# AI4Science-WestlakeU/safediffcon

Hardware: AMD Instinct MI355X
Metric: sampled control trajectories/sec (1000-step DDPM) (higher is better)
Workload: dtype f32; 1 GPU; C4: 2D smoke Unet3D_with_Conv3D dim=64 (1,2,4) state (B,32,7,64,64), B=64 per GPU, guided 1000-step DDPM, conformal quantile on; batch_per_gpu=64, global_batch=64, step=U-Net + guidance + posterior update of the whole batch, one hipGraph replay, parallelism=batch-sharded x1, no data-path collective, conv_precision=fp32

## Files before the change

### safediffcon_amd/csrc/sdc_conv.h

```cpp
#pragma once
#include "sdc_common.h"
#include <cstdlib>
#include <type_traits>

namespace sdcconv {


#ifdef SDC_KERNEL_EXPERIMENTS
inline int exp_env(const char* name) { const char* v = getenv(name); return v ? atoi(v) : 0; }
#else
constexpr int exp_env(const char*) { return 0; }
#endif


constexpr int BK = 16;
constexpr int NT = 256;

typedef float f32x16 __attribute__((ext_vector_type(16)));

typedef const __attribute__((address_space(1))) float* gfloat_p;
__device__ __forceinline__ gfloat_p uniform_ptr(const float* p) {
    const uint64_t u = reinterpret_cast<uint64_t>(p);
    const uint32_t lo = __builtin_amdgcn_readfirstlane((uint32_t)u);
    const uint32_t hi = __builtin_amdgcn_readfirstlane((uint32_t)(u >> 32));
    return (gfloat_p)(((uint64_t)hi << 32) | lo);
}
#define SDC_UNIFORM(v) __builtin_amdgcn_readfirstlane(v)
__device__ __forceinline__ float ld_sv(gfloat_p base, uint32_t byte_off) {
    typedef const __attribute__((address_space(1))) char* gchar_p;
    return *(gfloat_p)((gchar_p)base + byte_off);
}

struct ConvArgs {
    SdcConvDesc d;
    const float* x0;
    const float* x1;
    const float* wp;
    const float* bias;
    const float* res;
    float* y;
    int Ntot;
    int Ktot;
    int Cin;
    int lgD, lgH, lgW;
    int vec2;
    int ydense;
    const float* wg2;
    double* gn_part;
    int gn_G, gn_cpg, gn_nparts, gn_S;
    int ksplit;
    int64_t ypart_elems;
};

__device__ __forceinline__ int xcd_tile(int bid, int ntiles) {
    return (ntiles & 7) == 0 ? (bid & 7) * (ntiles >> 3) + (bid >> 3) : bid;
}

constexpr int W2_SK = 8;
constexpr int W2_BM = 64;
constexpr int W2_TILES = 64;
constexpr int W2_NBUF = 2;
constexpr int W2_ASZ = 16 * W2_SK * W2_BM, W2_BSZ = 16 * W2_SK * W2_TILES;
constexpr int W3S_TILES = 32;

inline int64_t span5(const int64_t* st, int b, int c, int dd, int h, int w) {
    return (int64_t)(b - 1) * st[0] + (int64_t)(c - 1) * st[1] + (int64_t)(dd - 1) * st[2] + (int64_t)(h - 1) * st[3] + (int64_t)(w - 1) * st[4];
}

bool wg2_ok(const SdcConvDesc& d, bool small);
bool wg3_ok(const SdcConvDesc& d, bool small);
int launch_wg2(const ConvArgs& a, hipStream_t s);
int wg2_ksplit(const SdcConvDesc& d);
int launch_wg3(const ConvArgs& a, hipStream_t s);
bool wg3s_ok(const SdcConvDesc& d, bool small);
bool wg2s_ok(const SdcConvDesc& d, bool small);
int launch_wg2s(const ConvArgs& a, hipStream_t s);
int launch_wg3s(const ConvArgs& a, hipStream_t s);

int f16_kc(int kD, int kH, int kW);
bool f16_faster(const SdcConvDesc& d);
bool f16_ok(const SdcConvDesc& d);
int f16_gnparts(const SdcConvDesc& d, int G);
const char* f16_name(const SdcConvDesc& d);
int launch_f16(const ConvArgs& a, const _Float16* wh, hipStream_t s, const int32_t* gexp = nullptr);
int pack_f16_tail(const float* w, float* tail, int64_t gap, int Cout, int Cin, int kD, int kH, int kW, hipStream_t s);

struct StemShape { int Hs, NG, NR, itemsB; size_t lds; };
StemShape stem_shape(const SdcConvDesc& d);
int launch_stem_f16(const SdcConvDesc& d, const float* x, const _Float16* wh, const float* bias, float* y, hipStream_t s);

int launch_stem_x3(const SdcConvDesc& d, const float* x, const __bf16* wb, const float* bias, float* y, hipStream_t s);

bool gemm_x3_covers(const SdcConvDesc& d);
int launch_gemm_x3(const SdcConvDesc& d, const float* x, const __bf16* wb, const float* bias, float* y, hipStream_t s);

int pw_x3_block(int K, int Cout);
int launch_pw_x3(const ConvArgs& a, hipStream_t s);

}
```

### safediffcon_amd/csrc/sdc_conv_gemm_x3.hip

```cpp
#include "sdc_conv.h"
#include "sdc_split3.h"

using namespace sdcconv;

namespace {

constexpr int GX_BM = 64, GX_BN = 256, GX_NT = 256;

struct GemmX3Args {
    const float* x;
    const __bf16* wb;
    const float* bias;
    float* y;
    int64_t xs[5], ys[5];
    int NP, oD, Cout, oH, W, lgW, iH, iW, lgIW;
    int pH, pW;
    int Hs, GR, NR, RP;
    int IMG;
    int RT, nrows, ntiles, mtiles, itemsB, nst;
    int plane;
};

template <int FORM> struct GxForm;
template <> struct GxForm<0> { static constexpr int TAPS = 16, NCB = 1, SS = 4, SH = 2, NPAR = 2; };
template <> struct GxForm<1> { static constexpr int TAPS = 4, NCB = 2, SS = 8, SH = 1, NPAR = 1; };
template <> struct GxForm<2> { static constexpr int TAPS = 1, NCB = 4, SS = 4, SH = 1, NPAR = 1; };

template <int FORM, int ITB>
__global__ __launch_bounds__(GX_NT) __attribute__((amdgpu_waves_per_eu(1))) SDC_NO_DS_MERGE void conv_gemm_x3_kernel(const GemmX3Args a) {
    using F = GxForm<FORM>;
    constexpr int TAPS = F::TAPS, NCB = F::NCB, SS = F::SS, SH = F::SH;
    constexpr int KS = NCB * TAPS;
    constexpr int NSUB = KS / SS;
    constexpr bool PREF = ITB <= 9;
    static_assert(NSUB * SS == KS, "whole sub-stages");
    constexpr int APC = SS * GX_BM * 32;
    constexpr int ASZ = 3 * APC;
    constexpr int NIA = 3 * SS * GX_BM * 2;
    constexpr int ITA = (NIA + GX_NT - 1) / GX_NT;
    extern __shared__ __attribute__((aligned(16))) char lds[];

    const int tid = threadIdx.x, lane = tid & 63, wave = tid >> 6;
    const int l31 = lane & 31, lh = lane >> 5;
    const int W = a.W, RP = a.RP;
    const int IMG = a.IMG, BIMG = 2 * NCB * IMG;
    const int PIMG = a.NR * RP * 16;
    const int logical = xcd_tile(blockIdx.x, a.ntiles * a.mtiles);
    const int mt = logical % a.mtiles, nt = logical / a.mtiles;
    const int m0 = mt * GX_BM;
    const int r0 = nt * a.RT;
    const int plane0 = r0 / a.oH, oh0 = r0 - plane0 * a.oH;

    int64_t bb[ITB];
    int bdst[ITB];
    bool bok[ITB];
#pragma unroll
    for (int k = 0; k < ITB; ++k) {
        const int it = tid + k * GX_NT;
        const int w = it & (a.iW - 1);
        const int rest = it >> a.lgIW;
        const int q = rest / a.NR, sr = rest - q * a.NR;
        const int g = sr / a.GR, sq = sr - g * a.GR;
        const int pl = plane0 + g, ih = SH * (g == 0 ? oh0 : 0) - a.pH + sq;
        const bool ok = it < a.itemsB && pl < a.NP && ih >= 0 && ih < a.iH;
        const int b = ok ? pl / a.oD : 0, od = ok ? pl % a.oD : 0, ihc = ok ? ih : 0;
        bok[k] = ok;
        bb[k] = (int64_t)b * a.xs[0] + (int64_t)od * a.xs[2] + (int64_t)ihc * a.xs[3] + (int64_t)w * a.xs[4]
                + (int64_t)((q >> 1) * 16 + (q & 1) * 8) * a.xs[1];
        int col;
        if (FORM == 0) col = (w & 1) * (PIMG / 16) + sr * RP + (w >> 1) + 1;
        else if (FORM == 1) col = sr * RP + w + 1;
        else col = sr * RP + w;
        bdst[k] = ASZ + q * IMG + col * 16;
    }
    int aoff[ITA];
#pragma unroll
    for (int k = 0; k < ITA; ++k) {
        const int it = tid + k * GX_NT;
        const int p = it / (SS * 2 * GX_BM), q = it - p * (SS * 2 * GX_BM);
        aoff[k] = it < NIA ? p * a.plane + mt * (a.nst * KS * GX_BM * 16) + q * 8 : 0;
    }

    float bv[ITB][8];
    uint4 av[ITA];
    auto load_a = [&](int st, int sub) {
        const int wst = (st * KS + sub * SS) * (GX_BM * 16);
#pragma unroll
        for (int k = 0; k < ITA; ++k) {
            uint4 v = make_uint4(0u, 0u, 0u, 0u);
            if (tid + k * GX_NT < NIA) v = *reinterpret_cast<const uint4*>(a.wb + wst + aoff[k]);
            av[k] = v;
        }
    };
    auto load_b = [&](int st) {
        const int64_t co = (int64_t)st * (NCB * 16) * a.xs[1];
#pragma unroll
        for (int k = 0; k < ITB; ++k) {
            const float* q = a.x + bb[k] + co;
#pragma unroll
            for (int i = 0; i < 8; ++i) { bv[k][i] = bok[k] ? *q : 0.0f; q += a.xs[1]; }
        }
    };
    auto store_a = [&]() {
#pragma unroll
        for (int k = 0; k < ITA; ++k)
            if (tid + k * GX_NT < NIA) *reinterpret_cast<uint4*>(lds + (tid + k * GX_NT) * 16) = av[k];
    };
    auto store_b = [&]() {
#pragma unroll
        for (int k = 0; k < ITB; ++k) {
            if (tid + k * GX_NT < a.itemsB) {
                bf16x8 h, m, l;
                split3x8(bv[k], h, m, l);
                *reinterpret_cast<bf16x8*>(lds + bdst[k]) = h;
                *reinterpret_cast<bf16x8*>(lds + bdst[k] + BIMG) = m;
                *reinterpret_cast<bf16x8*>(lds + bdst[k] + 2 * BIMG) = l;
            }
        }
    };

    if (FORM != 2) {
        const int nrows = 3 * 2 * NCB * F::NPAR * a.NR;
        for (int e = tid; e < 2 * nrows; e += GX_NT) {
            const int row = e >> 1;
            *reinterpret_cast<uint4*>(lds + ASZ + (row * RP + ((e & 1) ? RP - 1 : 0)) * 16) = make_uint4(0u, 0u, 0u, 0u);
        }
    }

    int bB[2];
#pragma unroll
    for (int j = 0; j < 2; ++j) {
        const int p = wave * 64 + 32 * j + l31;
        const bool pok = (p >> a.lgW) < a.RT && r0 + (p >> a.lgW) < a.nrows;
        const int rl = pok ? p >> a.lgW : 0, col = pok ? p & (W - 1) : 0;
        const int row = r0 + rl, pl = row / a.oH, oh = row - pl * a.oH, g = pl - plane0;
        const int slot = g * a.GR + SH * (oh - (g == 0 ? oh0 : 0));
        bB[j] = ASZ + (slot * RP + col + (FORM == 1 ? 1 - a.pW : 0)) * 16 + lh * IMG;
    }
    const int aoffr = l31 * 32 + 16 * lh;
    const int rowb = RP * 16;

    f32x16 acc[2][2], sm[2][2];
#pragma unroll
    for (int i = 0; i < 2; ++i)
#pragma unroll
        for (int j = 0; j < 2; ++j)
#pragma unroll
            for (int r = 0; r < 16; ++r) {
                acc[i][j][r] = 0.0f;
                sm[i][j][r] = 0.0f;
            }

    load_a(0, 0);
    if (PREF) load_b(0);
    for (int st = 0; st < a.nst; ++st) {
#pragma unroll
        for (int sub = 0; sub < NSUB; ++sub) {
            __syncthreads();
            store_a();
            if (sub == 0) {
                if (!PREF) load_b(st);
                store_b();
            }
            __syncthreads();
            if (sub + 1 < NSUB) load_a(st, sub + 1);
            else if (st + 1 < a.nst) {
                load_a(st + 1, 0);
                if (PREF) load_b(st + 1);
            }
#pragma unroll
            for (int sl = 0; sl < SS; ++sl) {
                const int ks = sub * SS + sl;
                const int cbk = ks / TAPS, tap = ks - cbk * TAPS;
                int tb = cbk * 2 * IMG;
                if (FORM == 0) {
                    const int kh = tap >> 2, kw = tap & 3;
                    tb += ((kw + 1) & 1) * PIMG + kh * rowb + ((kw + 1) >> 1) * 16;
                } else if (FORM == 1) {
                    tb += (tap >> 1) * rowb + (tap & 1) * 16;
                }
                bf16x8 af[2][3], bf[2][3];
#pragma unroll
                for (int i = 0; i < 2; ++i)
#pragma unroll
                    for (int p = 0; p < 3; ++p)
                        af[i][p] = *reinterpret_cast<const bf16x8*>(lds + p * APC + (sl * GX_BM + 32 * i) * 32 + aoffr);
#pragma unroll
                for (int j = 0; j < 2; ++j)
#pragma unroll
                    for (int p = 0; p < 3; ++p) bf[j][p] = *reinterpret_cast<const bf16x8*>(lds + bB[j] + tb + p * BIMG);
#pragma unroll
                for (int t = 0; t < 6; ++t)
#pragma unroll
                    for (int i = 0; i < 2; ++i)
#pragma unroll
                        for (int j = 0; j < 2; ++j) {
                            f32x16& c = t < 5 ? sm[i][j] : acc[i][j];
                            c = __builtin_amdgcn_mfma_f32_32x32x16_bf16(af[i][X3_PA[t]], bf[j][X3_PB[t]], c, 0, 0, 0);
                        }
            }
        }
    }

#pragma unroll
    for (int i = 0; i < 2; ++i)
#pragma unroll
        for (int j = 0; j < 2; ++j) acc[i][j] += sm[i][j];
    float bz[2][16];
#pragma unroll
    for (int i = 0; i < 2; ++i)
#pragma unroll
        for (int rr = 0; rr < 16; ++rr) bz[i][rr] = 0.0f;
    if (a.bias) {
#pragma unroll
        for (int i = 0; i < 2; ++i)
#pragma unroll
            for (int rr = 0; rr < 16; ++rr) bz[i][rr] = a.bias[m0 + 32 * i + 4 * lh + (rr & 3) + 8 * (rr >> 2)];
    }
#pragma unroll
    for (int j = 0; j < 2; ++j) {
        const int p = wave * 64 + 32 * j + l31;
        if ((p >> a.lgW) >= a.RT || r0 + (p >> a.lgW) >= a.nrows) continue;
        const int row = r0 + (p >> a.lgW), col = p & (W - 1);
        const int pl = row / a.oH, oh = row - pl * a.oH;
        const int b = pl / a.oD, od = pl - b * a.oD;
        float* yp = a.y + (int64_t)b * a.ys[0] + (int64_t)od * a.ys[2] + (int64_t)oh * a.ys[3] + (int64_t)col * a.ys[4]
                    + (int64_t)(m0 + 4 * lh) * a.ys[1];
#pragma unroll
        for (int i = 0; i < 2; ++i) {
#pragma unroll
            for (int rr = 0; rr < 16; ++rr)
                yp[(int64_t)(32 * i + (rr & 3) + 8 * (rr >> 2)) * a.ys[1]] = acc[i][j][rr] + bz[i][rr];
        }
    }
}

__global__ __launch_bounds__(256) void pack_gemm_x3_kernel(const float* __restrict__ wp, __bf16* __restrict__ out, int Cout, int Cin, int taps,
                                                           int ncb, int64_t n) {
    const int64_t e = (int64_t)blockIdx.x * 256 + threadIdx.x;
    if (e >= n) return;
    const int c16 = (int)(e & 15), col = (int)((e >> 4) & 63);
    int64_t r = e >> 10;
    const int KS = ncb * taps, nst = Cin / (16 * ncb);
    const int ks = (int)(r % KS); r /= KS;
    const int st = (int)(r % nst);
    const int mt = (int)(r / nst);
    const int cbk = ks / taps, tap = ks - cbk * taps;
    const int ci = (st * ncb + cbk) * 16 + c16, co = mt * 64 + col;
    __bf16 ph, pm, pl;
    split3(wp[((int64_t)tap * Cin + ci) * Cout + co], ph, pm, pl);
    out[e] = ph; out[n + e] = pm; out[2 * n + e] = pl;
}

int gx_ncb(int kH, int kW) { return kH == 4 && kW == 4 ? 1 : kH == 2 && kW == 2 ? 2 : kH == 1 && kW == 1 ? 4 : 0; }

struct GxShape { int form, RT, Hs, NG, GR, NR, RP, itemsB, IMG; size_t lds; };

GxShape gx_shape(const SdcConvDesc& d) {
    GxShape s{};
    s.form = d.kH == 4 ? 0 : d.kH == 2 ? 1 : 2;
    const int ncb = gx_ncb(d.kH, d.kW), npar = s.form == 0 ? 2 : 1, sh = s.form == 0 ? 2 : 1;
    const int ss = s.form == 1 ? 8 : 4;
    const int R = GX_BN / d.oW;
    const int maxit = (s.form == 0 ? 12 : 8) * GX_NT;
    auto fill = [&](int ng) {
        s.NG = ng;
        s.GR = sh * (s.Hs - 1) + d.kH;
        s.NR = s.NG * s.GR;
        s.RP = s.form == 0 ? d.iW / 2 + 2 : s.form == 1 ? d.iW + 2 : d.iW;
        s.IMG = npar * s.NR * s.RP * 16;
        s.itemsB = 2 * ncb * s.NR * d.iW;
        s.lds = (size_t)3 * ss * GX_BM * 32 + (size_t)3 * 2 * ncb * s.IMG;
        return s.itemsB <= maxit && s.lds <= 160u * 1024u;
    };
    if (d.oH < R) {
        s.Hs = d.oH;
        int ng = R / d.oH;
        while (!fill(ng) && ng > 1) --ng;
        s.RT = s.NG * d.oH;
    } else {
        s.Hs = R; s.RT = R;
        fill(d.oH % R == 0 ? 1 : 2);
    }
    return s;
}

}

namespace sdcconv {

bool gemm_x3_covers(const SdcConvDesc& d) {
    if (!(d.kD == 1 && d.sD == 1 && d.pD == 0 && d.uD == 1 && d.uH == 1 && d.uW == 1 && d.up_mode == 0 && d.oD == d.iD)) return false;
    if (!(d.B > 0 && d.oD > 0 && d.oH > 0 && d.Cin1 == 0 && d.Cout > 0 && d.Cout % 64 == 0)) return false;
    for (int i = 0; i < 5; ++i)
        if (d.rs[i] != 0 || d.x1s[i] != 0) return false;
    const int ncb = gx_ncb(d.kH, d.kW);
    if (ncb == 0 || d.Cin0 <= 0 || d.Cin0 % (16 * ncb) != 0) return false;
    if (d.kH == 4) {
        if (!(d.sH == 2 && d.sW == 2 && d.pH == 1 && d.pW == 1 && d.iH == 2 * d.oH && d.iW == 2 * d.oW)) return false;
    } else if (d.kH == 2) {
        if (!(d.sH == 1 && d.sW == 1 && (d.pH == 0 || d.pH == 1) && (d.pW == 0 || d.pW == 1) && d.iH == d.oH && d.iW == d.oW)) return false;
    } else {
        if (!(d.sH == 1 && d.sW == 1 && d.pH == 0 && d.pW == 0 && d.iH == d.oH && d.iW == d.oW)) return false;
    }
    if (!(d.oW == 16 || d.oW == 32 || d.oW == 64 || d.oW == 128)) return false;
    const GxShape s = gx_shape(d);
    return s.itemsB <= (s.form == 0 ? 12 : 8) * GX_NT && s.lds <= 160u * 1024u;
}

int launch_gemm_x3(const SdcConvDesc& d, const float* x, const __bf16* wb, const float* bias, float* y, hipStream_t s) {
    SDC_REQUIRE(reinterpret_cast<uintptr_t>(wb) % 16 == 0, SDC_EALIGN, "sdc_conv_gemm_x3: the packed weight buffer must be 16-byte aligned");
    const GxShape sh = gx_shape(d);
    const int ncb = gx_ncb(d.kH, d.kW);
    GemmX3Args a;
    a.x = x; a.wb = wb; a.bias = bias; a.y = y;
    for (int i = 0; i < 5; ++i) { a.xs[i] = d.x0s[i]; a.ys[i] = d.ys[i]; }
    a.NP = d.B * d.oD; a.oD = d.oD; a.Cout = d.Cout; a.oH = d.oH; a.W = d.oW; a.iH = d.iH; a.iW = d.iW;
    a.lgW = d.oW == 16 ? 4 : d.oW == 32 ? 5 : d.oW == 64 ? 6 : 7;
    a.lgIW = d.iW == d.oW ? a.lgW : a.lgW + 1;
    a.pH = d.pH; a.pW = d.pW;
    a.Hs = sh.Hs; a.GR = sh.GR; a.NR = sh.NR; a.RP = sh.RP; a.IMG = sh.IMG;
    const int64_t nrows = (int64_t)d.B * d.oD * d.oH;
    SDC_REQUIRE(nrows * d.oW < (1ll << 31), SDC_EINVAL, "sdc_conv_gemm_x3: too many output positions");
    const int64_t plane = (int64_t)d.kH * d.kW * d.Cin0 * d.Cout;
    SDC_REQUIRE(3 * plane < (1ll << 31), SDC_EINVAL, "sdc_conv_gemm_x3: weight too large");
    a.plane = (int)plane;
    a.nrows = (int)nrows; a.RT = sh.RT;
    a.ntiles = (a.nrows + sh.RT - 1) / sh.RT; a.mtiles = d.Cout / GX_BM;
    a.itemsB = sh.itemsB;
    a.nst = d.Cin0 / (16 * ncb);
    SDC_REQUIRE((int64_t)a.ntiles * a.mtiles < (1ll << 31), SDC_EINVAL, "sdc_conv_gemm_x3: grid too large");
    const dim3 grid((unsigned)(a.ntiles * a.mtiles));
#define GX_LAUNCH(FORM, ITB)                                                                                        \
    do {                                                                                                            \
        static std::atomic<uint64_t> attr{0};                                                                       \
        SDC_LDS_OPTIN(attr, (conv_gemm_x3_kernel<FORM, ITB>), 160 * 1024, "sdc_conv_gemm_x3");                      \
        hipLaunchKernelGGL((conv_gemm_x3_kernel<FORM, ITB>), grid, dim3(GX_NT), sh.lds, s, a);                      \
    } while (0)
    if (sh.form == 0) { if (sh.itemsB <= 9 * GX_NT) GX_LAUNCH(0, 9); else GX_LAUNCH(0, 12); }
    else if (sh.form == 1) { if (sh.itemsB <= 5 * GX_NT) GX_LAUNCH(1, 5); else GX_LAUNCH(1, 8); }
    else GX_LAUNCH(2, 8);
#undef GX_LAUNCH
    return sdc::check_launch("sdc_conv_gemm_x3");
}

}

extern "C" size_t sdc_pack_gemm_x3_bytes(int Cout, int Cin, int kH, int kW) {
    const int ncb = gx_ncb(kH, kW);
    if (ncb == 0 || Cout <= 0 || Cout % 64 != 0 || Cin <= 0 || Cin % (16 * ncb) != 0) return 0;
    return (size_t)3 * kH * kW * Cin * Cout * sizeof(__bf16);
}

extern "C" int sdc_pack_gemm_x3(const float* wp, void* out, int Cout, int Cin, int kH, int kW, void* stream) {
    SDC_REQUIRE(wp && out, SDC_ENULL, "sdc_pack_gemm_x3: null pointer");
    SDC_REQUIRE(sdc_pack_gemm_x3_bytes(Cout, Cin, kH, kW) > 0, SDC_EINVAL,
                "sdc_pack_gemm_x3: taps 4x4, 2x2 or 1x1, Cout a multiple of 64, Cin a multiple of 16 / 32 / 64 (got %dx%d, Cin %d, Cout %d)",
                kH, kW, Cin, Cout);
    const int64_t n = (int64_t)kH * kW * Cin * Cout;
    SDC_REQUIRE(n / 256 + 1 < (1ll << 31), SDC_EINVAL, "sdc_pack_gemm_x3: weight too large");
    hipLaunchKernelGGL(pack_gemm_x3_kernel, dim3((unsigned)((n + 255) / 256)), dim3(256), 0, sdc::as_stream(stream), wp,
                       reinterpret_cast<__bf16*>(out), Cout, Cin, kH * kW, gx_ncb(kH, kW), n);
    return sdc::check_launch("sdc_pack_gemm_x3");
}

static bool gemm_x3_faster(const SdcConvDesc& d) {
    const bool c64 = d.Cin0 == 64 && d.Cout == 64 && d.oH == 32 && d.oW == 32;
    const bool c128 = d.Cin0 == 128 && d.Cout == 128 && d.oH == 16 && d.oW == 16;
    return (d.kH == 4 || d.kH == 2) && (c64 || c128);
}

extern "C" int sdc_conv_gemm_x3_ok(const SdcConvDesc* dp) {
    return dp && gemm_x3_covers(*dp) && gemm_x3_faster(*dp) ? 1 : 0;
}

extern "C" int sdc_conv_gemm_x3(const SdcConvDesc* dp, const float* x, const void* wb, const float* bias, float* y, void* stream) {
    SDC_REQUIRE(dp && x && wb && y, SDC_ENULL, "sdc_conv_gemm_x3: null pointer");
    SDC_REQUIRE(gemm_x3_covers(*dp), SDC_EINVAL, "sdc_conv_gemm_x3: descriptor not covered: %dx%dx%d taps, stride %dx%dx%d, Cin %d+%d, Cout %d, "
                "residual %d, output %dx%dx%d", dp->kD, dp->kH, dp->kW, dp->sD, dp->sH, dp->sW, dp->Cin0, dp->Cin1, dp->Cout, (int)(dp->rs[1] != 0),
                dp->oD, dp->oH, dp->oW);
    return launch_gemm_x3(*dp, x, reinterpret_cast<const __bf16*>(wb), bias, y, sdc::as_stream(stream));
}
```

### safediffcon_amd/csrc/sdc_conv_stem_x3.hip

```cpp
#include "sdc_conv.h"
#include "sdc_conv_stem_tile.h"
#include "sdc_split3.h"

using namespace sdcconv;

namespace {

struct StemX3Args {
    STEM_TILE_ARGS(__bf16, wb)
    int plane;
};

template <int KH, int ITB>
__global__ __launch_bounds__(STEM_NT) __attribute__((amdgpu_waves_per_eu(1))) SDC_NO_DS_MERGE void conv_stem_x3_kernel(const StemX3Args a) {
    constexpr int TAPS = KH * 7;
    constexpr int NS = (TAPS + 1) / 2;
    constexpr int SS = KH == 7 ? 5 : NS;
    constexpr int NSUB = NS / SS;
    static_assert(NSUB * SS == NS, "whole sub-stages");
    constexpr int HH = KH - 1;
    constexpr int APC = SS * STEM_BM * 32;
    constexpr int ASZ = 3 * APC;
    constexpr int NIA = 3 * SS * STEM_BM * 2;
    constexpr int ITA = (NIA + STEM_NT - 1) / STEM_NT;
    extern __shared__ __attribute__((aligned(16))) char lds[];

    const int tid = threadIdx.x, lane = tid & 63, wave = tid >> 6;
    const int l31 = lane & 31, lh = lane >> 5;
    const int W = a.W, RP = W + 6;
    const int BIMG = a.NR * RP * 16;
    const StemTile t = stem_tile(a);
    const int m0 = t.m0, n0 = t.n0, r0 = t.r0, plane0 = t.plane0, oh0 = t.oh0;
    const int GR = a.Hs + HH;

    int64_t bb[ITB];
    int bod[ITB], bdst[ITB];
    bool bok[ITB];
#pragma unroll
    for (int k = 0; k < ITB; ++k) {
        const int it = tid + k * STEM_NT;
        const int w = it & (W - 1);
        const int sr = it >> a.lgW;
        int pl, ih;
        if (KH == 1) { const int row = r0 + sr; pl = row / a.oH; ih = row - pl * a.oH; }
        else { const int g = sr / GR, q = sr - g * GR; pl = plane0 + g; ih = (g == 0 ? oh0 : 0) - 3 + q; }
        const bool ok = it < a.itemsB && pl < a.B * a.oD && ih >= 0 && ih < a.oH;
        const int b = ok ? pl / a.oD : 0, od = ok ? pl % a.oD : 0, ihc = ok ? ih : 0;
        bok[k] = ok;
        bod[k] = od;
        bb[k] = (int64_t)b * a.xs[0] + (int64_t)od * a.xs[2] + (int64_t)ihc * a.xs[3] + (int64_t)w;
        bdst[k] = ASZ + (sr * RP + w + 3) * 16;
    }
    int aoff[ITA];
#pragma unroll
    for (int k = 0; k < ITA; ++k) {
        const int it = tid + k * STEM_NT;
        const int p = it / (SS * 2 * STEM_BM), q = it - p * (SS * 2 * STEM_BM);
        const int s = q / (2 * STEM_BM), r = q - s * (2 * STEM_BM);
        aoff[k] = it < NIA ? p * a.plane + (s * a.Cout + m0) * 16 + r * 8 : 0;
    }

    float bv[ITB][8];
    uint4 av[ITA];
    auto load_a = [&](int kd, int sub) {
        const int wst = (kd * NS + sub * SS) * a.Cout * 16;
#pragma unroll
        for (int k = 0; k < ITA; ++k) {
            uint4 v = make_uint4(0u, 0u, 0u, 0u);
            if (tid + k * STEM_NT < NIA) v = *reinterpret_cast<const uint4*>(a.wb + wst + aoff[k]);
            av[k] = v;
        }
    };
    auto load_b = [&](int kd) {
        const int dk = kd - a.kD / 2;
#pragma unroll
        for (int k = 0; k < ITB; ++k) {
            const int sd = bod[k] + dk;
            const bool ok = bok[k] && sd >= 0 && sd < a.oD;
            const float* q = a.x + bb[k] + (int64_t)dk * a.xs[2];
#pragma unroll
            for (int i = 0; i < 8; ++i) { bv[k][i] = (ok && i < a.Cin) ? *q : 0.0f; q += a.xs[1]; }
        }
    };
    auto store_a = [&]() {
#pragma unroll
        for (int k = 0; k < ITA; ++k)
            if (tid + k * STEM_NT < NIA) *reinterpret_cast<uint4*>(lds + (tid + k * STEM_NT) * 16) = av[k];
    };
    auto store_b = [&]() {
#pragma unroll
        for (int k = 0; k < ITB; ++k) {
            if (tid + k * STEM_NT < a.itemsB) {
                bf16x8 h, m, l;
                split3x8(bv[k], h, m, l);
                *reinterpret_cast<bf16x8*>(lds + bdst[k]) = h;
                *reinterpret_cast<bf16x8*>(lds + bdst[k] + BIMG) = m;
                *reinterpret_cast<bf16x8*>(lds + bdst[k] + 2 * BIMG) = l;
            }
        }
    };

    for (int e = tid; e < 3 * a.NR * 6; e += STEM_NT) {
        const int sr = e / 6, c = e - sr * 6;
        *reinterpret_cast<uint4*>(lds + ASZ + (sr * RP + (c < 3 ? c : W + c)) * 16) = make_uint4(0u, 0u, 0u, 0u);
    }

    int bA[2], bB[2], bC[2];
    constexpr int LAST_OFF = 16 * 6;
#pragma unroll
    for (int j = 0; j < 2; ++j) {
        const int p = wave * 64 + 32 * j + l31;
        const bool pok = n0 + p < a.Ntot;
        const int rl = pok ? p >> a.lgW : 0, col = pok ? p & (W - 1) : 0;
        int slot;
        if (KH == 1) slot = rl;
        else {
            const int row = r0 + rl, pl = row / a.oH, oh = row - pl * a.oH, g = pl - plane0;
            slot = g * GR + oh - (g == 0 ? oh0 : 0);
        }
        const int base = ASZ + (slot * RP + col) * 16;
        bA[j] = base + 16 * lh;
        bB[j] = base + lh * (RP * 16 - 16 * 6);
        bC[j] = lh ? ASZ - (HH * RP * 16 + LAST_OFF) : base;
    }
    const int aoffr = l31 * 32 + 16 * lh;
    const int rowb = RP * 16;

    f32x16 acc[2][2], sm[2][2];
#pragma unroll
    for (int i = 0; i < 2; ++i)
#pragma unroll
        for (int j = 0; j < 2; ++j)
#pragma unroll
            for (int r = 0; r < 16; ++r) {
                acc[i][j][r] = 0.0f;
                sm[i][j][r] = 0.0f;
            }

    load_a(0, 0);
    load_b(0);
    for (int kd = 0; kd < a.kD; ++kd) {
#pragma unroll
        for (int sub = 0; sub < NSUB; ++sub) {
            __syncthreads();
            store_a();
            if (sub == 0) store_b();
            __syncthreads();
            if (sub + 1 < NSUB) load_a(kd, sub + 1);
            else if (kd + 1 < a.kD) { load_a(kd + 1, 0); load_b(kd + 1); }
#pragma unroll
            for (int sl = 0; sl < SS; ++sl) {
                const int s = sub * SS + sl;
                const int t0 = 2 * s, kh = t0 / 7, kw = t0 - 7 * kh;
                const int tb = kh * rowb + kw * 16;
                bf16x8 af[2][3], bf[2][3];
#pragma unroll
                for (int i = 0; i < 2; ++i)
#pragma unroll
                    for (int p = 0; p < 3; ++p)
                        af[i][p] = *reinterpret_cast<const bf16x8*>(lds + p * APC + (sl * STEM_BM + 32 * i) * 32 + aoffr);
#pragma unroll
                for (int j = 0; j < 2; ++j) {
                    const int bs = (s == NS - 1) ? bC[j] : (kw == 6 ? bB[j] : bA[j]);
#pragma unroll
                    for (int p = 0; p < 3; ++p) bf[j][p] = *reinterpret_cast<const bf16x8*>(lds + bs + tb + p * BIMG);
                }
#pragma unroll
                for (int t = 0; t < 6; ++t)
#pragma unroll
                    for (int i = 0; i < 2; ++i)
#pragma unroll
                        for (int j = 0; j < 2; ++j) {
                            f32x16& c = t < 5 ? sm[i][j] : acc[i][j];
                            c = __builtin_amdgcn_mfma_f32_32x32x16_bf16(af[i][X3_PA[t]], bf[j][X3_PB[t]], c, 0, 0, 0);
                        }
            }
        }
    }

#pragma unroll
    for (int i = 0; i < 2; ++i)
#pragma unroll
        for (int j = 0; j < 2; ++j) acc[i][j] += sm[i][j];
    float bz[2][16];
#pragma unroll
    for (int i = 0; i < 2; ++i)
#pragma unroll
        for (int rr = 0; rr < 16; ++rr) bz[i][rr] = 0.0f;
    if (a.bias) {
#pragma unroll
        for (int i = 0; i < 2; ++i)
#pragma unroll
            for (int rr = 0; rr < 16; ++rr) bz[i][rr] = a.bias[m0 + 32 * i + 4 * lh + (rr & 3) + 8 * (rr >> 2)];
    }
#pragma unroll
    for (int j = 0; j < 2; ++j) {
        const int p = n0 + wave * 64 + 32 * j + l31;
        if (p >= a.Ntot) continue;
        const int row = p >> a.lgW, col = p & (W - 1);
        const int pl = row / a.oH, oh = row - pl * a.oH;
        const int b = pl / a.oD, od = pl - b * a.oD;
        float* yp = a.y + (int64_t)b * a.ys[0] + (int64_t)od * a.ys[2] + (int64_t)oh * a.ys[3] + (int64_t)col
                    + (int64_t)(m0 + 4 * lh) * a.ys[1];
#pragma unroll
        for (int i = 0; i < 2; ++i) {
#pragma unroll
            for (int rr = 0; rr < 16; ++rr)
                yp[(int64_t)(32 * i + (rr & 3) + 8 * (rr >> 2)) * a.ys[1]] = acc[i][j][rr] + bz[i][rr];
        }
    }
}

__global__ __launch_bounds__(256) void pack_stem_x3_kernel(const float* __restrict__ w, __bf16* __restrict__ out, int Cout, int Cin, int kD,
                                                           int taps, int NS, int64_t n) {
    const int64_t e = (int64_t)blockIdx.x * 256 + threadIdx.x;
    if (e >= n) return;
    const int ci = (int)(e & 7), h = (int)((e >> 3) & 1);
    int64_t r = e >> 4;
    const int co = (int)(r % Cout); r /= Cout;
    const int s = (int)(r % NS);
    const int kd = (int)(r / NS);
    const int t = 2 * s + h;
    const float v = (ci < Cin && t < taps) ? w[(((int64_t)co * Cin + ci) * kD + kd) * taps + t] : 0.0f;
    __bf16 ph, pm, pl;
    split3(v, ph, pm, pl);
    out[e] = ph; out[n + e] = pm; out[2 * n + e] = pl;
}

}

namespace sdcconv {

int launch_stem_x3(const SdcConvDesc& d, const float* x, const __bf16* wb, const float* bias, float* y, hipStream_t s) {
    SDC_REQUIRE(reinterpret_cast<uintptr_t>(wb) % 16 == 0, SDC_EALIGN, "sdc_conv_stem_x3: the packed weight buffer must be 16-byte aligned");
    const StemShape sh = stem_shape(d);
    const int NS = (d.kH * 7 + 1) / 2, SS = d.kH == 7 ? 5 : NS;
    const size_t lds = (size_t)3 * SS * STEM_BM * 32 + (size_t)3 * sh.NR * (d.oW + 6) * 16;
    SDC_REQUIRE(sh.itemsB <= 8 * STEM_NT && lds <= 160u * 1024u, SDC_EINVAL, "sdc_conv_stem_x3: staging of %d positions / %zu bytes of LDS",
                sh.itemsB, lds);
    StemX3Args a;
    a.wb = wb;
    if (const int rc = stem_fill_args("sdc_conv_stem_x3", d, sh, x, bias, y, a)) return rc;
    const int64_t plane = (int64_t)d.kD * NS * d.Cout * 16;
    SDC_REQUIRE(3 * plane < (1ll << 31), SDC_EINVAL, "sdc_conv_stem_x3: weight too large");
    a.plane = (int)plane;
    STEM_LAUNCH(conv_stem_x3_kernel, "sdc_conv_stem_x3");
    return sdc::check_launch("sdc_conv_stem_x3");
}

}

extern "C" size_t sdc_pack_stem_x3_bytes(int Cout, int Cin, int kD, int kH, int kW) {
    return 3 * sdc_pack_stem_f16_bytes(Cout, Cin, kD, kH, kW);
}

extern "C" int sdc_pack_stem_x3(const float* w, void* out, int Cout, int Cin, int kD, int kH, int kW, void* stream) {
    SDC_REQUIRE(w && out, SDC_ENULL, "sdc_pack_stem_x3: null pointer");
    SDC_REQUIRE(sdc_pack_stem_x3_bytes(Cout, Cin, kD, kH, kW) > 0, SDC_EINVAL,
                "sdc_pack_stem_x3: taps 1x1x7, 1x7x7 or 7x7x7 and 1 <= Cin <= 8 (got %dx%dx%d, Cin %d, Cout %d)", kD, kH, kW, Cin, Cout);
    const int NS = (kH * 7 + 1) / 2;
    const int64_t n = (int64_t)kD * NS * Cout * 16;
    SDC_REQUIRE(n / 256 + 1 < (1ll << 31), SDC_EINVAL, "sdc_pack_stem_x3: weight too large");
    hipLaunchKernelGGL(pack_stem_x3_kernel, dim3((unsigned)((n + 255) / 256)), dim3(256), 0, sdc::as_stream(stream), w,
                       reinterpret_cast<__bf16*>(out), Cout, Cin, kD, kH * 7, NS, n);
    return sdc::check_launch("sdc_pack_stem_x3");
}
```

Before: 0.3134 trajectories/s.

## Make gemm_x3 conv persistent with cross-tile prefetch; add debug ablation variants

The gemm_x3 convolution kernel becomes a persistent loop over tiles. The grid size comes from a ta_grid helper, and on the last K stage of each tile the kernel prefetches the next tile's weights, input items and fragment bases. This hides the load prologue between tiles and cuts block launch overhead. The change also adds compile-time DBG template variants, selected by an environment variable only under SDC_KERNEL_EXPERIMENTS, that skip loads, stores or barriers to profile the gemm_x3 and stem_x3 kernels. The persistent loop adds register pressure from holding the next tile's state, and it depends on the grid sizing being right.

```diff
diff --git a/safediffcon_amd/csrc/sdc_conv.h b/safediffcon_amd/csrc/sdc_conv.h
--- a/safediffcon_amd/csrc/sdc_conv.h
+++ b/safediffcon_amd/csrc/sdc_conv.h
@@ -56,6 +56,14 @@
     return (ntiles & 7) == 0 ? (bid & 7) * (ntiles >> 3) + (bid >> 3) : bid;
 }
 
+constexpr int GD_STORE = 1;
+constexpr int GD_SPLIT = 2;
+constexpr int GD_STA = 4;
+constexpr int GD_BAR = 8;
+constexpr int GD_FRAG = 16;
+constexpr int GD_LOAD = 32;
+[[maybe_unused]] constexpr int GD_MFMA_ONLY = 63;
+
 constexpr int W2_SK = 8;
 constexpr int W2_BM = 64;
 constexpr int W2_TILES = 64;
diff --git a/safediffcon_amd/csrc/sdc_conv_gemm_x3.hip b/safediffcon_amd/csrc/sdc_conv_gemm_x3.hip
--- a/safediffcon_amd/csrc/sdc_conv_gemm_x3.hip
+++ b/safediffcon_amd/csrc/sdc_conv_gemm_x3.hip
@@ -2,6 +2,8 @@
 #include "sdc_split3.h"
 
 using namespace sdcconv;
+
+namespace sdc { int ta_grid(const char* entry, int64_t nblk, unsigned* grid); }
 
 namespace {
 
@@ -26,7 +28,7 @@
 template <> struct GxForm<1> { static constexpr int TAPS = 4, NCB = 2, SS = 8, SH = 1, NPAR = 1; };
 template <> struct GxForm<2> { static constexpr int TAPS = 1, NCB = 4, SS = 4, SH = 1, NPAR = 1; };
 
-template <int FORM, int ITB>
+template <int FORM, int ITB, int DBG = 0>
 __global__ __launch_bounds__(GX_NT) __attribute__((amdgpu_waves_per_eu(1))) SDC_NO_DS_MERGE void conv_gemm_x3_kernel(const GemmX3Args a) {
     using F = GxForm<FORM>;
     constexpr int TAPS = F::TAPS, NCB = F::NCB, SS = F::SS, SH = F::SH;
@@ -45,28 +47,45 @@
     const int W = a.W, RP = a.RP;
     const int IMG = a.IMG, BIMG = 2 * NCB * IMG;
     const int PIMG = a.NR * RP * 16;
-    const int logical = xcd_tile(blockIdx.x, a.ntiles * a.mtiles);
-    const int mt = logical % a.mtiles, nt = logical / a.mtiles;
-    const int m0 = mt * GX_BM;
-    const int r0 = nt * a.RT;
-    const int plane0 = r0 / a.oH, oh0 = r0 - plane0 * a.oH;
+    const int total = a.ntiles * a.mtiles;
+    const bool dbg_dead = DBG != 0 && a.NP < 0;
+
+    struct Tile { int mt, r0, plane0, oh0; };
+    auto tile_of = [&](int phys) {
+        const int logical = xcd_tile(phys, total);
+        Tile t;
+        t.mt = logical % a.mtiles;
+        t.r0 = (logical / a.mtiles) * a.RT;
+        t.plane0 = t.r0 / a.oH;
+        t.oh0 = t.r0 - t.plane0 * a.oH;
+        return t;
+    };
 
     int64_t bb[ITB];
     int bdst[ITB];
     bool bok[ITB];
+    auto set_items = [&](const Tile& t) {
+#pragma unroll
+        for (int k = 0; k < ITB; ++k) {
+            const int it = tid + k * GX_NT;
+            const int w = it & (a.iW - 1);
+            const int rest = it >> a.lgIW;
+            const int q = rest / a.NR, sr = rest - q * a.NR;
+            const int g = sr / a.GR, sq = sr - g * a.GR;
+            const int pl = t.plane0 + g, ih = SH * (g == 0 ? t.oh0 : 0) - a.pH + sq;
+            const bool ok = it < a.itemsB && pl < a.NP && ih >= 0 && ih < a.iH;
+            const int b = ok ? pl / a.oD : 0, od = ok ? pl % a.oD : 0, ihc = ok ? ih : 0;
+            bok[k] = ok;
+            bb[k] = (int64_t)b * a.xs[0] + (int64_t)od * a.xs[2] + (int64_t)ihc * a.xs[3] + (int64_t)w * a.xs[4]
+                    + (int64_t)((q >> 1) * 16 + (q & 1) * 8) * a.xs[1];
+        }
+    };
 #pragma unroll
     for (int k = 0; k < ITB; ++k) {
         const int it = tid + k * GX_NT;
         const int w = it & (a.iW - 1);
         const int rest = it >> a.lgIW;
         const int q = rest / a.NR, sr = rest - q * a.NR;
-        const int g = sr / a.GR, sq = sr - g * a.GR;
-        const int pl = plane0 + g, ih = SH * (g == 0 ? oh0 : 0) - a.pH + sq;
-        const bool ok = it < a.itemsB && pl < a.NP && ih >= 0 && ih < a.iH;
-        const int b = ok ? pl / a.oD : 0, od = ok ? pl % a.oD : 0, ihc = ok ? ih : 0;
-        bok[k] = ok;
-        bb[k] = (int64_t)b * a.xs[0] + (int64_t)od * a.xs[2] + (int64_t)ihc * a.xs[3] + (int64_t)w * a.xs[4]
-                + (int64_t)((q >> 1) * 16 + (q & 1) * 8) * a.xs[1];
         int col;
         if (FORM == 0) col = (w & 1) * (PIMG / 16) + sr * RP + (w >> 1) + 1;
         else if (FORM == 1) col = sr * RP + w + 1;
@@ -78,17 +97,18 @@
     for (int k = 0; k < ITA; ++k) {
         const int it = tid + k * GX_NT;
         const int p = it / (SS * 2 * GX_BM), q = it - p * (SS * 2 * GX_BM);
-        aoff[k] = it < NIA ? p * a.plane + mt * (a.nst * KS * GX_BM * 16) + q * 8 : 0;
+        aoff[k] = it < NIA ? p * a.plane + q * 8 : 0;
     }
 
     float bv[ITB][8];
     uint4 av[ITA];
-    auto load_a = [&](int st, int sub) {
-        const int wst = (st * KS + sub * SS) * (GX_BM * 16);
+    auto load_a = [&](int mt, int st, int sub) {
+        const int wst = mt * (a.nst * KS * GX_BM * 16) + (st * KS + sub * SS) * (GX_BM * 16);
 #pragma unroll
         for (int k = 0; k < ITA; ++k) {
             uint4 v = make_uint4(0u, 0u, 0u, 0u);
-            if (tid + k * GX_NT < NIA) v = *reinterpret_cast<const uint4*>(a.wb + wst + aoff[k]);
+            if (!(DBG & GD_LOAD) || dbg_dead)
+                if (tid + k * GX_NT < NIA) v = *reinterpret_cast<const uint4*>(a.wb + wst + aoff[k]);
             av[k] = v;
         }
     };
@@ -97,16 +117,19 @@
 #pragma unroll
         for (int k = 0; k < ITB; ++k) {
             const float* q = a.x + bb[k] + co;
-#pragma unroll
-            for (int i = 0; i < 8; ++i) { bv[k][i] = bok[k] ? *q : 0.0f; q += a.xs[1]; }
+            const bool ok = bok[k] && (!(DBG & GD_LOAD) || dbg_dead);
+#pragma unroll
+            for (int i = 0; i < 8; ++i) { bv[k][i] = ok ? *q : 0.0f; q += a.xs[1]; }
         }
     };
     auto store_a = [&]() {
+        if ((DBG & GD_STA) && !dbg_dead) return;
 #pragma unroll
         for (int k = 0; k < ITA; ++k)
             if (tid + k * GX_NT < NIA) *reinterpret_cast<uint4*>(lds + (tid + k * GX_NT) * 16) = av[k];
     };
     auto store_b = [&]() {
+        if ((DBG & GD_SPLIT) && !dbg_dead) return;
 #pragma unroll
         for (int k = 0; k < ITB; ++k) {
             if (tid + k * GX_NT < a.itemsB) {
@@ -118,6 +141,9 @@
             }
         }
     };
+    auto barrier = [&]() {
+        if constexpr (!(DBG & GD_BAR)) __syncthreads();
+    };
 
     if (FORM != 2) {
         const int nrows = 3 * 2 * NCB * F::NPAR * a.NR;
@@ -127,111 +153,145 @@
         }
     }
 
-    int bB[2];
-#pragma unroll
-    for (int j = 0; j < 2; ++j) {
-        const int p = wave * 64 + 32 * j + l31;
-        const bool pok = (p >> a.lgW) < a.RT && r0 + (p >> a.lgW) < a.nrows;
-        const int rl = pok ? p >> a.lgW : 0, col = pok ? p & (W - 1) : 0;
-        const int row = r0 + rl, pl = row / a.oH, oh = row - pl * a.oH, g = pl - plane0;
-        const int slot = g * a.GR + SH * (oh - (g == 0 ? oh0 : 0));
-        bB[j] = ASZ + (slot * RP + col + (FORM == 1 ? 1 - a.pW : 0)) * 16 + lh * IMG;
-    }
+    auto frag_bases = [&](const Tile& t, int (&dst)[2]) {
+#pragma unroll
+        for (int j = 0; j < 2; ++j) {
+            const int p = wave * 64 + 32 * j + l31;
+            const bool pok = (p >> a.lgW) < a.RT && t.r0 + (p >> a.lgW) < a.nrows;
+            const int rl = pok ? p >> a.lgW : 0, col = pok ? p & (W - 1) : 0;
+            const int row = t.r0 + rl, pl = row / a.oH, oh = row - pl * a.oH, g = pl - t.plane0;
+            const int slot = g * a.GR + SH * (oh - (g == 0 ? t.oh0 : 0));
+            dst[j] = ASZ + (slot * RP + col + (FORM == 1 ? 1 - a.pW : 0)) * 16 + lh * IMG;
+        }
+    };
     const int aoffr = l31 * 32 + 16 * lh;
     const int rowb = RP * 16;
 
-    f32x16 acc[2][2], sm[2][2];
-#pragma unroll
-    for (int i = 0; i < 2; ++i)
-#pragma unroll
-        for (int j = 0; j < 2; ++j)
-#pragma unroll
-            for (int r = 0; r < 16; ++r) {
-                acc[i][j][r] = 0.0f;
-                sm[i][j][r] = 0.0f;
+    int phys = blockIdx.x;
+    Tile cur = tile_of(phys), nxt = cur;
+    int bB[2], nbB[2] = {0, 0};
+    set_items(cur);
+    frag_bases(cur, bB);
+    load_a(cur.mt, 0, 0);
+    if (PREF) load_b(0);
+
+    for (;;) {
+        const int nphys = phys + (int)gridDim.x;
+        const bool more = nphys < total;
+        f32x16 acc[2][2], sm[2][2];
+#pragma unroll
+        for (int i = 0; i < 2; ++i)
+#pragma unroll
+            for (int j = 0; j < 2; ++j)
+#pragma unroll
+                for (int r = 0; r < 16; ++r) {
+                    acc[i][j][r] = 0.0f;
+                    sm[i][j][r] = 0.0f;
+                }
+
+        for (int st = 0; st < a.nst; ++st) {
+#pragma unroll
+            for (int sub = 0; sub < NSUB; ++sub) {
+                barrier();
+                store_a();
+                if (sub == 0) {
+                    if (!PREF) load_b(st);
+                    store_b();
+                }
+                barrier();
+                if (sub + 1 < NSUB) load_a(cur.mt, st, sub + 1);
+                else if (st + 1 < a.nst) {
+                    load_a(cur.mt, st + 1, 0);
+                    if (PREF) load_b(st + 1);
+                } else if (more) {
+                    nxt = tile_of(nphys);
+                    set_items(nxt);
+                    frag_bases(nxt, nbB);
+                    load_a(nxt.mt, 0, 0);
+                    if (PREF) load_b(0);
+                }
+#pragma unroll
+                for (int sl = 0; sl < SS; ++sl) {
+                    const int ks = sub * SS + sl;
+                    const int cbk = ks / TAPS, tap = ks - cbk * TAPS;
+                    int tb = cbk * 2 * IMG;
+                    if (FORM == 0) {
+                        const int kh = tap >> 2, kw = tap & 3;
+                        tb += ((kw + 1) & 1) * PIMG + kh * rowb + ((kw + 1) >> 1) * 16;
+                    } else if (FORM == 1) {
+                        tb += (tap >> 1) * rowb + (tap & 1) * 16;
+                    }
+                    bf16x8 af[2][3], bf[2][3];
+                    if constexpr (DBG & GD_FRAG) {
+                        const uint4 u = make_uint4((unsigned)tid * 0x9E3779B9u, (unsigned)tid, (unsigned)lane, 0x3F803F80u);
+#pragma unroll
+                        for (int i = 0; i < 2; ++i)
+#pragma unroll
+                            for (int p = 0; p < 3; ++p) {
+                                af[i][p] = __builtin_bit_cast(bf16x8, u);
+                                bf[i][p] = __builtin_bit_cast(bf16x8, u);
+                            }
+                    } else {
+#pragma unroll
+                        for (int i = 0; i < 2; ++i)
+#pragma unroll
+                            for (int p = 0; p < 3; ++p)
+                                af[i][p] = *reinterpret_cast<const bf16x8*>(lds + p * APC + (sl * GX_BM + 32 * i) * 32 + aoffr);
+#pragma unroll
+                        for (int j = 0; j < 2; ++j)
+#pragma unroll
+                            for (int p = 0; p < 3; ++p) bf[j][p] = *reinterpret_cast<const bf16x8*>(lds + bB[j] + tb + p * BIMG);
+                    }
+#pragma unroll
+                    for (int t = 0; t < 6; ++t)
+#pragma unroll
+                        for (int i = 0; i < 2; ++i)
+#pragma unroll
+                            for (int j = 0; j < 2; ++j) {
+                                f32x16& c = t < 5 ? sm[i][j] : acc[i][j];
+                                c = __builtin_amdgcn_mfma_f32_32x32x16_bf16(af[i][X3_PA[t]], bf[j][X3_PB[t]], c, 0, 0, 0);
+                            }
+                }
             }
-
-    load_a(0, 0);
-    if (PREF) load_b(0);
-    for (int st = 0; st < a.nst; ++st) {
-#pragma unroll
-        for (int sub = 0; sub < NSUB; ++sub) {
-            __syncthreads();
-            store_a();
-            if (sub == 0) {
-                if (!PREF) load_b(st);
-                store_b();
+        }
+
+#pragma unroll
+        for (int i = 0; i < 2; ++i)
+#pragma unroll
+            for (int j = 0; j < 2; ++j) acc[i][j] += sm[i][j];
+        const int m0 = cur.mt * GX_BM, r0 = cur.r0;
+        float bz[2][16];
+#pragma unroll
+        for (int i = 0; i < 2; ++i)
+#pragma unroll
+            for (int rr = 0; rr < 16; ++rr) bz[i][rr] = 0.0f;
+        if (a.bias) {
+#pragma unroll
+            for (int i = 0; i < 2; ++i)
+#pragma unroll
+                for (int rr = 0; rr < 16; ++rr) bz[i][rr] = a.bias[m0 + 32 * i + 4 * lh + (rr & 3) + 8 * (rr >> 2)];
+        }
+#pragma unroll
+        for (int j = 0; j < 2; ++j) {
+            const int p = wave * 64 + 32 * j + l31;
+            if ((p >> a.lgW) >= a.RT || r0 + (p >> a.lgW) >= a.nrows) continue;
+            if ((DBG & GD_STORE) && !dbg_dead) continue;
+            const int row = r0 + (p >> a.lgW), col = p & (W - 1);
+            const int pl = row / a.oH, oh = row - pl * a.oH;
+            const int b = pl / a.oD, od = pl - b * a.oD;
+            float* yp = a.y + (int64_t)b * a.ys[0] + (int64_t)od * a.ys[2] + (int64_t)oh * a.ys[3] + (int64_t)col * a.ys[4]
+                        + (int64_t)(m0 + 4 * lh) * a.ys[1];
+#pragma unroll
+            for (int i = 0; i < 2; ++i) {
+#pragma unroll
+                for (int rr = 0; rr < 16; ++rr)
+                    yp[(int64_t)(32 * i + (rr & 3) + 8 * (rr >> 2)) * a.ys[1]] = acc[i][j][rr] + bz[i][rr];
             }
-            __syncthreads();
-            if (sub + 1 < NSUB) load_a(st, sub + 1);
-            else if (st + 1 < a.nst) {
-                load_a(st + 1, 0);
-                if (PREF) load_b(st + 1);
-            }
-#pragma unroll
-            for (int sl = 0; sl < SS; ++sl) {
-                const int ks = sub * SS + sl;
-                const int cbk = ks / TAPS, tap = ks - cbk * TAPS;
-                int tb = cbk * 2 * IMG;
-                if (FORM == 0) {
-                    const int kh = tap >> 2, kw = tap & 3;
-                    tb += ((kw + 1) & 1) * PIMG + kh * rowb + ((kw + 1) >> 1) * 16;
-                } else if (FORM == 1) {
-                    tb += (tap >> 1) * rowb + (tap & 1) * 16;
-                }
-                bf16x8 af[2][3], bf[2][3];
-#pragma unroll
-                for (int i = 0; i < 2; ++i)
-#pragma unroll
-                    for (int p = 0; p < 3; ++p)
-                        af[i][p] = *reinterpret_cast<const bf16x8*>(lds + p * APC + (sl * GX_BM + 32 * i) * 32 + aoffr);
-#pragma unroll
-                for (int j = 0; j < 2; ++j)
-#pragma unroll
-                    for (int p = 0; p < 3; ++p) bf[j][p] = *reinterpret_cast<const bf16x8*>(lds + bB[j] + tb + p * BIMG);
-#pragma unroll
-                for (int t = 0; t < 6; ++t)
-#pragma unroll
-                    for (int i = 0; i < 2; ++i)
-#pragma unroll
-                        for (int j = 0; j < 2; ++j) {
-                            f32x16& c = t < 5 ? sm[i][j] : acc[i][j];
-                            c = __builtin_amdgcn_mfma_f32_32x32x16_bf16(af[i][X3_PA[t]], bf[j][X3_PB[t]], c, 0, 0, 0);
-                        }
-            }
-        }
-    }
-
-#pragma unroll
-    for (int i = 0; i < 2; ++i)
-#pragma unroll
-        for (int j = 0; j < 2; ++j) acc[i][j] += sm[i][j];
-    float bz[2][16];
-#pragma unroll
-    for (int i = 0; i < 2; ++i)
-#pragma unroll
-        for (int rr = 0; rr < 16; ++rr) bz[i][rr] = 0.0f;
-    if (a.bias) {
-#pragma unroll
-        for (int i = 0; i < 2; ++i)
-#pragma unroll
-            for (int rr = 0; rr < 16; ++rr) bz[i][rr] = a.bias[m0 + 32 * i + 4 * lh + (rr & 3) + 8 * (rr >> 2)];
-    }
-#pragma unroll
-    for (int j = 0; j < 2; ++j) {
-        const int p = wave * 64 + 32 * j + l31;
-        if ((p >> a.lgW) >= a.RT || r0 + (p >> a.lgW) >= a.nrows) continue;
-        const int row = r0 + (p >> a.lgW), col = p & (W - 1);
-        const int pl = row / a.oH, oh = row - pl * a.oH;
-        const int b = pl / a.oD, od = pl - b * a.oD;
-        float* yp = a.y + (int64_t)b * a.ys[0] + (int64_t)od * a.ys[2] + (int64_t)oh * a.ys[3] + (int64_t)col * a.ys[4]
-                    + (int64_t)(m0 + 4 * lh) * a.ys[1];
-#pragma unroll
-        for (int i = 0; i < 2; ++i) {
-#pragma unroll
-            for (int rr = 0; rr < 16; ++rr)
-                yp[(int64_t)(32 * i + (rr & 3) + 8 * (rr >> 2)) * a.ys[1]] = acc[i][j][rr] + bz[i][rr];
-        }
+        }
+        if (!more) break;
+        phys = nphys;
+        cur = nxt;
+        bB[0] = nbB[0]; bB[1] = nbB[1];
     }
 }
 
@@ -330,13 +390,35 @@
     a.itemsB = sh.itemsB;
     a.nst = d.Cin0 / (16 * ncb);
     SDC_REQUIRE((int64_t)a.ntiles * a.mtiles < (1ll << 31), SDC_EINVAL, "sdc_conv_gemm_x3: grid too large");
-    const dim3 grid((unsigned)(a.ntiles * a.mtiles));
-#define GX_LAUNCH(FORM, ITB)                                                                                        \
+    unsigned nwg = 0;
+    if (const int rc = sdc::ta_grid("sdc_conv_gemm_x3", (int64_t)a.ntiles * a.mtiles, &nwg)) return rc;
+    const dim3 grid(nwg);
+#define GX_LAUNCH(...)                                                                                              \
     do {                                                                                                            \
         static std::atomic<uint64_t> attr{0};                                                                       \
-        SDC_LDS_OPTIN(attr, (conv_gemm_x3_kernel<FORM, ITB>), 160 * 1024, "sdc_conv_gemm_x3");                      \
-        hipLaunchKernelGGL((conv_gemm_x3_kernel<FORM, ITB>), grid, dim3(GX_NT), sh.lds, s, a);                      \
+        SDC_LDS_OPTIN(attr, (conv_gemm_x3_kernel<__VA_ARGS__>), 160 * 1024, "sdc_conv_gemm_x3");                    \
+        hipLaunchKernelGGL((conv_gemm_x3_kernel<__VA_ARGS__>), grid, dim3(GX_NT), sh.lds, s, a);                    \
     } while (0)
+#ifdef SDC_KERNEL_EXPERIMENTS
+    const int dbg = getenv("SDC_CONVX3_DBG") ? atoi(getenv("SDC_CONVX3_DBG")) : 0;
+    if (dbg && ((sh.form == 0 && sh.itemsB <= 9 * GX_NT) || (sh.form == 1 && sh.itemsB <= 5 * GX_NT))) {
+#define GX_DBG_CASE(D)                                                                                              \
+        case D:                                                                                                     \
+            if (sh.form == 0) GX_LAUNCH(0, 9, D); else GX_LAUNCH(1, 5, D);                                          \
+            break
+        switch (dbg) {
+            GX_DBG_CASE(GD_STORE);
+            GX_DBG_CASE(GD_SPLIT);
+            GX_DBG_CASE(GD_STA);
+            GX_DBG_CASE(GD_BAR);
+            GX_DBG_CASE(GD_FRAG);
+            GX_DBG_CASE(GD_LOAD);
+            default: if (sh.form == 0) GX_LAUNCH(0, 9, GD_MFMA_ONLY); else GX_LAUNCH(1, 5, GD_MFMA_ONLY); break;
+        }
+#undef GX_DBG_CASE
+        return sdc::check_launch("sdc_conv_gemm_x3");
+    }
+#endif
     if (sh.form == 0) { if (sh.itemsB <= 9 * GX_NT) GX_LAUNCH(0, 9); else GX_LAUNCH(0, 12); }
     else if (sh.form == 1) { if (sh.itemsB <= 5 * GX_NT) GX_LAUNCH(1, 5); else GX_LAUNCH(1, 8); }
     else GX_LAUNCH(2, 8);
diff --git a/safediffcon_amd/csrc/sdc_conv_stem_x3.hip b/safediffcon_amd/csrc/sdc_conv_stem_x3.hip
--- a/safediffcon_amd/csrc/sdc_conv_stem_x3.hip
+++ b/safediffcon_amd/csrc/sdc_conv_stem_x3.hip
@@ -11,7 +11,7 @@
     int plane;
 };
 
-template <int KH, int ITB>
+template <int KH, int ITB, int DBG = 0>
 __global__ __launch_bounds__(STEM_NT) __attribute__((amdgpu_waves_per_eu(1))) SDC_NO_DS_MERGE void conv_stem_x3_kernel(const StemX3Args a) {
     constexpr int TAPS = KH * 7;
     constexpr int NS = (TAPS + 1) / 2;
@@ -32,6 +32,7 @@
     const StemTile t = stem_tile(a);
     const int m0 = t.m0, n0 = t.n0, r0 = t.r0, plane0 = t.plane0, oh0 = t.oh0;
     const int GR = a.Hs + HH;
+    const bool dbg_dead = DBG != 0 && a.B < 0;
 
     int64_t bb[ITB];
     int bod[ITB], bdst[ITB];
@@ -67,7 +68,8 @@
 #pragma unroll
         for (int k = 0; k < ITA; ++k) {
             uint4 v = make_uint4(0u, 0u, 0u, 0u);
-            if (tid + k * STEM_NT < NIA) v = *reinterpret_cast<const uint4*>(a.wb + wst + aoff[k]);
+            if (!(DBG & GD_LOAD) || dbg_dead)
+                if (tid + k * STEM_NT < NIA) v = *reinterpret_cast<const uint4*>(a.wb + wst + aoff[k]);
             av[k] = v;
         }
     };
@@ -76,18 +78,20 @@
 #pragma unroll
         for (int k = 0; k < ITB; ++k) {
             const int sd = bod[k] + dk;
-            const bool ok = bok[k] && sd >= 0 && sd < a.oD;
+            const bool ok = bok[k] && sd >= 0 && sd < a.oD && (!(DBG & GD_LOAD) || dbg_dead);
             const float* q = a.x + bb[k] + (int64_t)dk * a.xs[2];
 #pragma unroll
             for (int i = 0; i < 8; ++i) { bv[k][i] = (ok && i < a.Cin) ? *q : 0.0f; q += a.xs[1]; }
         }
     };
     auto store_a = [&]() {
+        if ((DBG & GD_STA) && !dbg_dead) return;
 #pragma unroll
         for (int k = 0; k < ITA; ++k)
             if (tid + k * STEM_NT < NIA) *reinterpret_cast<uint4*>(lds + (tid + k * STEM_NT) * 16) = av[k];
     };
     auto store_b = [&]() {
+        if ((DBG & GD_SPLIT) && !dbg_dead) return;
 #pragma unroll
         for (int k = 0; k < ITB; ++k) {
             if (tid + k * STEM_NT < a.itemsB) {
@@ -98,6 +102,10 @@
                 *reinterpret_cast<bf16x8*>(lds + bdst[k] + 2 * BIMG) = l;
             }
         }
+    };
+
+    auto barrier = [&]() {
+        if constexpr (!(DBG & GD_BAR)) __syncthreads();
     };
 
     for (int e = tid; e < 3 * a.NR * 6; e += STEM_NT) {
@@ -142,10 +150,10 @@
     for (int kd = 0; kd < a.kD; ++kd) {
 #pragma unroll
         for (int sub = 0; sub < NSUB; ++sub) {
-            __syncthreads();
+            barrier();
             store_a();
             if (sub == 0) store_b();
-            __syncthreads();
+            barrier();
             if (sub + 1 < NSUB) load_a(kd, sub + 1);
             else if (kd + 1 < a.kD) { load_a(kd + 1, 0); load_b(kd + 1); }
 #pragma unroll
@@ -154,16 +162,27 @@
                 const int t0 = 2 * s, kh = t0 / 7, kw = t0 - 7 * kh;
                 const int tb = kh * rowb + kw * 16;
                 bf16x8 af[2][3], bf[2][3];
-#pragma unroll
-                for (int i = 0; i < 2; ++i)
-#pragma unroll
-                    for (int p = 0; p < 3; ++p)
-                        af[i][p] = *reinterpret_cast<const bf16x8*>(lds + p * APC + (sl * STEM_BM + 32 * i) * 32 + aoffr);
-#pragma unroll
-                for (int j = 0; j < 2; ++j) {
-                    const int bs = (s == NS - 1) ? bC[j] : (kw == 6 ? bB[j] : bA[j]);
-#pragma unroll
-                    for (int p = 0; p < 3; ++p) bf[j][p] = *reinterpret_cast<const bf16x8*>(lds + bs + tb + p * BIMG);
+                if constexpr (DBG & GD_FRAG) {
+                    const uint4 u = make_uint4((unsigned)tid * 0x9E3779B9u, (unsigned)tid, (unsigned)lane, 0x3F803F80u);
+#pragma unroll
+                    for (int i = 0; i < 2; ++i)
+#pragma unroll
+                        for (int p = 0; p < 3; ++p) {
+                            af[i][p] = __builtin_bit_cast(bf16x8, u);
+                            bf[i][p] = __builtin_bit_cast(bf16x8, u);
+                        }
+                } else {
+#pragma unroll
+                    for (int i = 0; i < 2; ++i)
+#pragma unroll
+                        for (int p = 0; p < 3; ++p)
+                            af[i][p] = *reinterpret_cast<const bf16x8*>(lds + p * APC + (sl * STEM_BM + 32 * i) * 32 + aoffr);
+#pragma unroll
+                    for (int j = 0; j < 2; ++j) {
+                        const int bs = (s == NS - 1) ? bC[j] : (kw == 6 ? bB[j] : bA[j]);
+#pragma unroll
+                        for (int p = 0; p < 3; ++p) bf[j][p] = *reinterpret_cast<const bf16x8*>(lds + bs + tb + p * BIMG);
+                    }
                 }
 #pragma unroll
                 for (int t = 0; t < 6; ++t)
@@ -197,6 +216,7 @@
     for (int j = 0; j < 2; ++j) {
         const int p = n0 + wave * 64 + 32 * j + l31;
         if (p >= a.Ntot) continue;
+        if ((DBG & GD_STORE) && !dbg_dead) continue;
         const int row = p >> a.lgW, col = p & (W - 1);
         const int pl = row / a.oH, oh = row - pl * a.oH;
         const int b = pl / a.oD, od = pl - b * a.oD;
@@ -244,6 +264,28 @@
     const int64_t plane = (int64_t)d.kD * NS * d.Cout * 16;
     SDC_REQUIRE(3 * plane < (1ll << 31), SDC_EINVAL, "sdc_conv_stem_x3: weight too large");
     a.plane = (int)plane;
+#ifdef SDC_KERNEL_EXPERIMENTS
+    const int dbg = getenv("SDC_CONVX3_DBG") ? atoi(getenv("SDC_CONVX3_DBG")) : 0;
+    if (dbg && d.kH == 7 && sh.itemsB > 2 * STEM_NT && sh.itemsB <= 4 * STEM_NT) {
+#define SX_DBG_LAUNCH(D)                                                                                            \
+        do {                                                                                                        \
+            static std::atomic<uint64_t> attr{0};                                                                   \
+            SDC_LDS_OPTIN(attr, (conv_stem_x3_kernel<7, 4, D>), 160 * 1024, "sdc_conv_stem_x3");                    \
+            hipLaunchKernelGGL((conv_stem_x3_kernel<7, 4, D>), dim3((unsigned)(a.ntiles * a.mtiles)), dim3(STEM_NT), lds, s, a); \
+        } while (0)
+        switch (dbg) {
+            case GD_STORE: SX_DBG_LAUNCH(GD_STORE); break;
+            case GD_SPLIT: SX_DBG_LAUNCH(GD_SPLIT); break;
+            case GD_STA: SX_DBG_LAUNCH(GD_STA); break;
+            case GD_BAR: SX_DBG_LAUNCH(GD_BAR); break;
+            case GD_FRAG: SX_DBG_LAUNCH(GD_FRAG); break;
+            case GD_LOAD: SX_DBG_LAUNCH(GD_LOAD); break;
+            default: SX_DBG_LAUNCH(GD_MFMA_ONLY); break;
+        }
+#undef SX_DBG_LAUNCH
+        return sdc::check_launch("sdc_conv_stem_x3");
+    }
+#endif
     STEM_LAUNCH(conv_stem_x3_kernel, "sdc_conv_stem_x3");
     return sdc::check_launch("sdc_conv_stem_x3");
 }
```

Result: no change. 0.3137 trajectories/s, median of 4 (+0.1%).
